# Infini-AI-Lab/Sequoia

Measured on NVIDIA H100. Metric: decoded tokens/sec (mean accepted len/step in config.accepted_tokens_per_step), Sequoia tree speculative decoding, 68m->7B Llama (config c2 unless --config says otherwise), higher is better.
Workload: dtype f16

## Files before the change

sequoia_b200/csrc/sq_gemm.cu:

```cuda
#include <cstdio>
#include <cstdlib>

#include "sq_common.cuh"
#include "sq_ptx.cuh"

struct sq_gemm_plan {
  CUtensorMap tm_a, tm_w;
  __half* c;
  int ldc, n_max, N, K, bn, split, stages, mc, pdl, tiled, epi, n_out;
  int* err_flag;
};

namespace sq {

struct GemmArgs {
  __half* c;
  int ldc, n, N, K, kb_per_split;
  int tiled, kb_total;
  int m0;
  int epi, n_out;
  int* err_flag;
};

constexpr int G_BK = 64;
constexpr int G_THREADS = 384;
constexpr int G_CONSUMER_WARPS = 8;

template <int BN, int STAGES, int SPLIT>
struct GemmSmem {
  static constexpr int A_BYTES = 128 * 128;
  static constexpr int W_BYTES = BN * 128;
  static constexpr int STAGE_BYTES = A_BYTES + ((W_BYTES + 1023) / 1024) * 1024;
  static constexpr int OFF_BAR = STAGES * STAGE_BYTES;
  static constexpr int OFF_RED = OFF_BAR + 256;
  static constexpr int R_STRIDE = BN + 4;
  static constexpr int RED_BYTES = SPLIT > 1 ? 128 * R_STRIDE * 4 : 0;
  static constexpr int TOTAL = OFF_RED + RED_BYTES;
};

__device__ __forceinline__ void tma_load_2d_mc(uint32_t dst, const CUtensorMap* tm, uint32_t bar, int c0, int c1, uint16_t mask) {
  asm volatile(
      "cp.async.bulk.tensor.2d.shared::cluster.global.mbarrier::complete_tx::bytes.multicast::cluster [%0], [%1, {%4, %5}], [%2], %3;" ::"r"(dst),
      "l"(tm), "r"(bar), "h"(mask), "r"(c0), "r"(c1)
      : "memory");
}

template <int BN, int STAGES, int SPLIT, int MC>
__global__ void __launch_bounds__(G_THREADS, 1)
    gemm_tn_kernel(const __grid_constant__ CUtensorMap tm_a, const __grid_constant__ CUtensorMap tm_w, GemmArgs g) {
  using SM = GemmSmem<BN, STAGES, SPLIT>;
  constexpr int NCH = BN / 64;
  extern __shared__ __align__(1024) uint8_t smem_raw[];
  uint8_t* smem = smem_raw + ((1024u - (ptx::smem_u32(smem_raw) & 1023u)) & 1023u);
  const int tid = threadIdx.x, warp = tid >> 5, lane = tid & 31;
  const int n0 = blockIdx.x * BN;
  const int ks = blockIdx.y;
  const int mcr = (MC > 1) ? (int)(blockIdx.x % MC) : 0;
  const int kb0 = ks * g.kb_per_split;
  const int nkb = g.kb_per_split;
  const uint32_t s_base = ptx::smem_u32(smem);
  const uint32_t bar_full = s_base + SM::OFF_BAR, bar_empty = bar_full + 8 * STAGES;

  if (tid == 0) {
#pragma unroll
    for (int s = 0; s < STAGES; ++s) {
      ptx::mbar_init(bar_full + 8 * s, 1);
      ptx::mbar_init(bar_empty + 8 * s, G_CONSUMER_WARPS * MC);
    }
    ptx::fence_barrier_init();
  }
  __syncthreads();
  if (MC > 1)
    asm volatile("barrier.cluster.arrive.release.aligned;\n\tbarrier.cluster.wait.acquire.aligned;" ::: "memory");

  if (warp < 4) {
    if (tid == 0) {
      asm volatile("griddepcontrol.launch_dependents;" ::: "memory");
      const int pre = nkb < STAGES ? nkb : STAGES;
      for (int kb = 0; kb < pre; ++kb) {
        const uint32_t sa = s_base + kb * SM::STAGE_BYTES, sw = sa + SM::A_BYTES;
        ptx::mbar_expect_tx(bar_full + 8 * kb, SM::A_BYTES + SM::W_BYTES);
        if (g.tiled) ptx::tma_load_2d(sw, &tm_w, bar_full + 8 * kb, 0, ((int)blockIdx.x * g.kb_total + kb0 + kb) * BN);
        else ptx::tma_load_2d(sw, &tm_w, bar_full + 8 * kb, (kb0 + kb) * G_BK, n0);
      }
      asm volatile("griddepcontrol.wait;" ::: "memory");
      int stage = 0;
      uint32_t phase = 0;
      for (int kb = 0; kb < nkb; ++kb) {
        const uint32_t sa = s_base + stage * SM::STAGE_BYTES, sw = sa + SM::A_BYTES;
        if (kb >= pre) {
          ptx::mbar_wait_one(bar_empty + 8 * stage, phase ^ 1, g.err_flag, 11);
          ptx::mbar_expect_tx(bar_full + 8 * stage, SM::A_BYTES + SM::W_BYTES);
          if (g.tiled) ptx::tma_load_2d(sw, &tm_w, bar_full + 8 * stage, 0, ((int)blockIdx.x * g.kb_total + kb0 + kb) * BN);
          else ptx::tma_load_2d(sw, &tm_w, bar_full + 8 * stage, (kb0 + kb) * G_BK, n0);
        }
        if (MC == 1) ptx::tma_load_2d(sa, &tm_a, bar_full + 8 * stage, (kb0 + kb) * G_BK, g.m0);
        else tma_load_2d_mc(sa + mcr * (SM::A_BYTES / MC), &tm_a, bar_full + 8 * stage, (kb0 + kb) * G_BK, g.m0 + mcr * (128 / MC),
                            (uint16_t)(((1u << MC) - 1u) << (MC * ks)));
        if (++stage == STAGES) { stage = 0; phase ^= 1; }
      }
    }
  } else {
    const int wg = (warp >> 2) - 1;
    float acc[NCH][32];
#pragma unroll
    for (int c = 0; c < NCH; ++c)
#pragma unroll
      for (int e = 0; e < 32; ++e) acc[c][e] = 0.f;
    auto release = [&](int s) {
      if (lane == 0) {
        if (MC == 1) asm volatile("mbarrier.arrive.shared::cta.b64 _, [%0];" ::"r"(bar_empty + 8 * s) : "memory");
        else
          for (int r = 0; r < MC; ++r) ptx::mbar_arrive_cluster(bar_empty + 8 * s, (uint32_t)(MC * ks + r));
      }
    };
    int stage = 0, prev = -1;
    uint32_t phase = 0;
    for (int kb = 0; kb < nkb; ++kb) {
      ptx::mbar_wait(bar_full + 8 * stage, phase, g.err_flag, 12);
      const uint32_t sa = s_base + stage * SM::STAGE_BYTES + wg * 8192, sw = s_base + stage * SM::STAGE_BYTES + SM::A_BYTES;
      ptx::wgmma_fence();
#pragma unroll
      for (int k = 0; k < G_BK / 16; ++k)
#pragma unroll
        for (int c = 0; c < NCH; ++c)
          ptx::wgmma_ss<0>(acc[c], gmma_desc(sa + k * 32, 16, 1024), gmma_desc(sw + c * 8192 + k * 32, 16, 1024), 1);
      ptx::wgmma_commit();
      asm volatile("wgmma.wait_group.sync.aligned 1;" ::: "memory");
      if (prev >= 0) release(prev);
      prev = stage;
      if (++stage == STAGES) { stage = 0; phase ^= 1; }
    }
    ptx::wgmma_wait_all();
    if (prev >= 0) release(prev);
    const int rbase = wg * 64 + (warp & 3) * 16 + (lane >> 2), q2 = 2 * (lane & 3);
    if (SPLIT == 1 && g.epi == 1) {
#pragma unroll
      for (int h = 0; h < 2; ++h) {
        const int row = rbase + 8 * h;
        if (row >= g.n) continue;
        __half* orow = g.c + (int64_t)(g.m0 + row) * g.ldc;
#pragma unroll
        for (int c = 0; c < NCH; ++c)
#pragma unroll
          for (int j = 0; j < 8; ++j) {
            if ((j & 3) >= 2) continue;
            const int ob = (n0 + c * 64 + (j >> 2) * 32) / 2;
            if (ob >= g.n_out) continue;
            __half o[2];
#pragma unroll
            for (int e = 0; e < 2; ++e) {
              const float x = h2f(f2h(acc[c][4 * j + 2 * h + e]));
              const __half act = f2h(x / (1.0f + expf(-x)));
              o[e] = f2h(h2f(act) * h2f(f2h(acc[c][4 * (j + 2) + 2 * h + e])));
            }
            *reinterpret_cast<__half2*>(orow + ob + (j & 3) * 8 + q2) = __halves2half2(o[0], o[1]);
          }
      }
    } else if (SPLIT == 1) {
#pragma unroll
      for (int h = 0; h < 2; ++h) {
        const int row = rbase + 8 * h;
        if (row >= g.n) continue;
        __half* crow = g.c + (int64_t)(g.m0 + row) * g.ldc + n0;
#pragma unroll
        for (int c = 0; c < NCH; ++c)
#pragma unroll
          for (int j = 0; j < 8; ++j)
            if (n0 + c * 64 + j * 8 < g.N)
              *reinterpret_cast<__half2*>(crow + c * 64 + j * 8 + q2) =
                  __floats2half2_rn(acc[c][4 * j + 2 * h], acc[c][4 * j + 2 * h + 1]);
      }
    } else {
      constexpr int RPC = 128 / SPLIT;
#pragma unroll
      for (int h = 0; h < 2; ++h) {
        const int row = rbase + 8 * h;
        uint32_t dst;
        asm volatile("mapa.shared::cluster.u32 %0, %1, %2;" : "=r"(dst) : "r"(s_base + SM::OFF_RED), "r"((uint32_t)mcr + MC * (row / RPC)));
        dst += (uint32_t)((ks * RPC + row % RPC) * SM::R_STRIDE * 4);
#pragma unroll
        for (int c = 0; c < NCH; ++c)
#pragma unroll
          for (int j = 0; j < 8; ++j)
            asm volatile("st.shared::cluster.v2.f32 [%0], {%1, %2};" ::"r"(dst + (c * 64 + j * 8 + q2) * 4),
                         "f"(acc[c][4 * j + 2 * h]), "f"(acc[c][4 * j + 2 * h + 1])
                         : "memory");
      }
    }
  }
  __syncthreads();

  if (MC > 1 || SPLIT > 1)
    asm volatile("barrier.cluster.arrive.release.aligned;\n\tbarrier.cluster.wait.acquire.aligned;" ::: "memory");

  if (SPLIT > 1) {
    constexpr int RPC = 128 / SPLIT;
    constexpr int CPR = BN / 4;
    const float* red = reinterpret_cast<const float*>(smem + SM::OFF_RED);
    for (int i = tid; i < RPC * CPR; i += G_THREADS) {
      const int lr = i / CPR, cc = i % CPR;
      const int row = ks * RPC + lr;
      if (row >= g.n) continue;
      float4 acc = make_float4(0.f, 0.f, 0.f, 0.f);
#pragma unroll
      for (int s = 0; s < SPLIT; ++s) {
        const float4 o = *reinterpret_cast<const float4*>(red + (s * RPC + lr) * SM::R_STRIDE + cc * 4);
        acc.x += o.x; acc.y += o.y; acc.z += o.z; acc.w += o.w;
      }
      const __half2 lo = __floats2half2_rn(acc.x, acc.y), hi = __floats2half2_rn(acc.z, acc.w);
      uint2 pk;
      pk.x = *reinterpret_cast<const uint32_t*>(&lo);
      pk.y = *reinterpret_cast<const uint32_t*>(&hi);
      *reinterpret_cast<uint2*>(g.c + (int64_t)(g.m0 + row) * g.ldc + n0 + cc * 4) = pk;
    }
  }
}

}

using namespace sq;

typedef CUresult (*PFN_tmapEncodeTiledG)(CUtensorMap*, CUtensorMapDataType, cuuint32_t, void*, const cuuint64_t*,
                                         const cuuint64_t*, const cuuint32_t*, const cuuint32_t*, CUtensorMapInterleave,
                                         CUtensorMapSwizzle, CUtensorMapL2promotion, CUtensorMapFloatOOBfill);

static int encode_2d(CUtensorMap* tm, const void* base, uint64_t inner, uint64_t outer, uint64_t pitch_bytes,
                     uint32_t box_inner, uint32_t box_outer, CUtensorMapL2promotion prom) {
  static PFN_tmapEncodeTiledG fn = nullptr;
  if (!fn) {
    void* p = nullptr;
    cudaDriverEntryPointQueryResult qres;
    if (cudaGetDriverEntryPoint("cuTensorMapEncodeTiled", &p, cudaEnableDefault, &qres) == cudaSuccess &&
        qres == cudaDriverEntryPointSuccess)
      fn = (PFN_tmapEncodeTiledG)p;
  }
  if (!fn) { set_error("cuTensorMapEncodeTiled unavailable"); return SQ_ERR_CUDA; }
  cuuint64_t dims[2] = {inner, outer};
  cuuint64_t strides[1] = {pitch_bytes};
  cuuint32_t box[2] = {box_inner, box_outer};
  cuuint32_t estr[2] = {1, 1};
  CUresult r = fn(tm, CU_TENSOR_MAP_DATA_TYPE_FLOAT16, 2, const_cast<void*>(base), dims, strides, box, estr,
                  CU_TENSOR_MAP_INTERLEAVE_NONE, CU_TENSOR_MAP_SWIZZLE_128B, prom, CU_TENSOR_MAP_FLOAT_OOB_FILL_NONE);
  if (r != CUDA_SUCCESS) { set_error("cuTensorMapEncodeTiled failed: %d", (int)r); return SQ_ERR_CUDA; }
  return SQ_OK;
}

static int sm_count() {
  static int n_sm = 0;
  if (!n_sm) {
    int dev = 0;
    if (cudaGetDevice(&dev) != cudaSuccess || cudaDeviceGetAttribute(&n_sm, cudaDevAttrMultiProcessorCount, dev) != cudaSuccess ||
        n_sm <= 0) {
      cudaGetLastError();
      n_sm = 132;
    }
  }
  return n_sm;
}

static void choose_tiles(sq_gemm_plan* p, bool allow_split) {
  const int N = p->N, kb = p->K / 64;
  const int n_sm = sm_count();
  const int cands[] = {256, 192, 128, 64};
  int best_bn = 128, best_split = 1, best_mc = 1;
  double best_score = -1.0;
  for (int bn : cands) {
    const int tiles = (N + bn - 1) / bn;
    for (int split : {1, 2, 4}) {
      if (kb % split || (split > 1 && !allow_split)) continue;
      if (split > 1 && (bn > 128 || N % bn)) continue;
      const int ctas = tiles * split;
      if (ctas > n_sm) continue;
      for (int mc : {1, 2}) {
        if (mc == 2 && tiles % 2) continue;
        const double a_share = 128.0 / mc, share = bn / (bn + a_share);
        double score = ctas * share;
        if (split > 1) score *= 0.85;
        if (score > best_score) { best_score = score; best_bn = bn; best_split = split; best_mc = mc; }
      }
    }
  }
  p->bn = best_bn; p->split = best_split; p->mc = best_mc;
}

static void pick_tiles(sq_gemm_plan* p) {
  const int kb = p->K / 64;
  const bool allow_split = p->epi == 0;
  choose_tiles(p, allow_split);
  const char* force = getenv("SQ_GEMM_FORCE");
  if (force) {
    int fb = 0, fs = 0, fm = 1;
    const int nf = sscanf(force, "%d,%d,%d", &fb, &fs, &fm);
    const bool bn_ok = fb == 64 || fb == 128 || fb == 192 || fb == 256;
    if (nf >= 2 && bn_ok && (fs == 1 || fs == 2 || fs == 4) && kb % fs == 0 && (fm == 1 || fm == 2) &&
        !(fs > 1 && (fb > 128 || p->N % fb || !allow_split)) && !(fm == 2 && ((p->N + fb - 1) / fb) % 2)) {
      p->bn = fb; p->split = fs; p->mc = fm;
    }
  }
}

extern "C" int sq_gemm_pick_tiles(int N, int K, int* bn, int* split, int* mc) { return sq_gemm_pick_tiles_ex(N, K, 0, bn, split, mc); }

extern "C" int sq_gemm_pick_tiles_ex(int N, int K, int flags, int* bn, int* split, int* mc) {
  SQ_CHECK_ARG(K % 64 == 0 && N % 32 == 0, "sq_gemm_pick_tiles: K %% 64, N %% 32");
  sq_gemm_plan p{};
  p.N = N; p.K = K; p.epi = (flags & SQ_GEMM_SWIGLU) ? 1 : 0;
  pick_tiles(&p);
  *bn = p.bn; *split = p.split; *mc = p.mc;
  return SQ_OK;
}

static int plan_create(sq_gemm_plan** plan, const sq_half* a, int lda, int n_max, const sq_half* w, int N, int K, sq_half* c,
                       int ldc, int* err_flag, int flags);

extern "C" int sq_gemm_plan_create(sq_gemm_plan** plan, const sq_half* a, int lda, int n_max, const sq_half* w, int N,
                                   int K, sq_half* c, int ldc, int* err_flag) {
  return plan_create(plan, a, lda, n_max, w, N, K, c, ldc, err_flag, 0);
}

extern "C" int sq_gemm_plan_create_tiled(sq_gemm_plan** plan, const sq_half* a, int lda, int n_max, const sq_half* w_tiled,
                                         int N, int K, sq_half* c, int ldc, int* err_flag) {
  return plan_create(plan, a, lda, n_max, w_tiled, N, K, c, ldc, err_flag, SQ_GEMM_TILED);
}

extern "C" int sq_gemm_plan_create_ex(sq_gemm_plan** plan, const sq_half* a, int lda, int n_max, const sq_half* w, int N,
                                      int K, sq_half* c, int ldc, int* err_flag, int flags) {
  return plan_create(plan, a, lda, n_max, w, N, K, c, ldc, err_flag, flags);
}

static int plan_create(sq_gemm_plan** plan, const sq_half* a, int lda, int n_max, const sq_half* w, int N, int K, sq_half* c,
                       int ldc, int* err_flag, int flags) {
  const int tiled = (flags & SQ_GEMM_TILED) ? 1 : 0;
  SQ_CHECK_ARG(plan && a && w && c, "sq_gemm_plan_create: null pointer");
  SQ_CHECK_ARG(K % 64 == 0 && N % 32 == 0 && lda % 8 == 0 && ldc % 8 == 0, "sq_gemm_plan_create: K %% 64, N %% 32");
  sq_gemm_plan* p = new sq_gemm_plan();
  p->c = (__half*)c; p->ldc = ldc; p->n_max = n_max; p->N = N; p->K = K; p->err_flag = err_flag;
  p->tiled = tiled; p->epi = (flags & SQ_GEMM_SWIGLU) ? 1 : 0; p->n_out = p->epi ? N / 2 : 0;
  if (p->epi) SQ_CHECK_ARG(N % 32 == 0, "sq_gemm_plan_create: SwiGLU needs N %% 32 == 0");
  pick_tiles(p);
  {
    p->pdl = pdl_enabled() ? 1 : 0;
  }
  p->stages = p->split > 1 ? 4 : (p->bn == 256 ? 4 : p->bn == 192 ? 5 : p->bn == 128 ? 6 : 8);
  int rc = encode_2d(&p->tm_a, a, (uint64_t)K, (uint64_t)n_max, (uint64_t)lda * 2, 64, (uint32_t)(128 / p->mc),
                     CU_TENSOR_MAP_L2_PROMOTION_L2_128B);
  if (!rc) {
    if (tiled) rc = encode_2d(&p->tm_w, w, 64, (uint64_t)((N + p->bn - 1) / p->bn) * (uint64_t)(K / 64) * (uint64_t)p->bn, 128, 64,
                              (uint32_t)p->bn, CU_TENSOR_MAP_L2_PROMOTION_L2_256B);
    else rc = encode_2d(&p->tm_w, w, (uint64_t)K, (uint64_t)N, (uint64_t)K * 2, 64, (uint32_t)p->bn, CU_TENSOR_MAP_L2_PROMOTION_L2_256B);
  }
  if (rc) { delete p; return rc; }
  *plan = p;
  return SQ_OK;
}

extern "C" int sq_gemm_plan_destroy(sq_gemm_plan* plan) {
  delete plan;
  return SQ_OK;
}

template <int BN, int STAGES, int SPLIT, int MC>
static int launch_gemm(sq_gemm_plan* p, GemmArgs& g, cudaStream_t st) {
  using SM = GemmSmem<BN, STAGES, SPLIT>;
  constexpr int smem = SM::TOTAL + 1024;
  static_assert(smem <= 227 * 1024, "shared memory budget");
  static bool attr = false;
  if (!attr) {
    cudaError_t e = cudaFuncSetAttribute(gemm_tn_kernel<BN, STAGES, SPLIT, MC>, cudaFuncAttributeMaxDynamicSharedMemorySize, smem);
    if (e != cudaSuccess) { set_error("sq_gemm: smem attr: %s", cudaGetErrorString(e)); return SQ_ERR_CUDA; }
    attr = true;
  }
  cudaLaunchConfig_t cfg{};
  cfg.gridDim = dim3((p->N + BN - 1) / BN, SPLIT, 1);
  cfg.blockDim = dim3(G_THREADS);
  cfg.dynamicSmemBytes = smem;
  cfg.stream = st;
  cudaLaunchAttribute at[2];
  at[0].id = cudaLaunchAttributeClusterDimension;
  at[0].val.clusterDim.x = MC;
  at[0].val.clusterDim.y = SPLIT;
  at[0].val.clusterDim.z = 1;
  cfg.attrs = at;
  cfg.numAttrs = 1;
  if (p->pdl) {
    at[1].id = cudaLaunchAttributeProgrammaticStreamSerialization;
    at[1].val.programmaticStreamSerializationAllowed = 1;
    cfg.numAttrs = 2;
  }
  cudaError_t e = cudaLaunchKernelEx(&cfg, gemm_tn_kernel<BN, STAGES, SPLIT, MC>, p->tm_a, p->tm_w, g);
  if (e != cudaSuccess) { set_error("sq_gemm: launch failed: %s", cudaGetErrorString(e)); return SQ_ERR_CUDA; }
  SQ_CHECK_LAUNCH("sq_gemm");
  return SQ_OK;
}

static int run_tile(sq_gemm_plan* plan, GemmArgs& g, cudaStream_t st) {
  const int bn = plan->bn, sp = plan->split, mc = plan->mc;
#define SQ_G(BN_, ST_, SP_, MC_) if (bn == BN_ && sp == SP_ && mc == MC_) return launch_gemm<BN_, ST_, SP_, MC_>(plan, g, st)
  SQ_G(256, 4, 1, 1); SQ_G(256, 4, 1, 2);
  SQ_G(192, 5, 1, 1); SQ_G(192, 5, 1, 2);
  SQ_G(128, 6, 1, 1); SQ_G(128, 6, 1, 2); SQ_G(128, 4, 2, 1); SQ_G(128, 4, 4, 1); SQ_G(128, 4, 2, 2); SQ_G(128, 4, 4, 2);
  SQ_G(64, 8, 1, 1); SQ_G(64, 8, 1, 2); SQ_G(64, 4, 2, 1); SQ_G(64, 4, 4, 1); SQ_G(64, 4, 2, 2); SQ_G(64, 4, 4, 2);
#undef SQ_G
  set_error("sq_gemm_run: no kernel for bn=%d split=%d mc=%d", bn, sp, mc);
  return SQ_ERR_UNSUPPORTED;
}

extern "C" int sq_gemm_run(sq_gemm_plan* plan, int n, void* stream) { return sq_gemm_run_at(plan, n, 0, nullptr, 0, stream); }

extern "C" int sq_gemm_run_at(sq_gemm_plan* plan, int n, int a_row0, sq_half* c, int ldc, void* stream) {
  SQ_CHECK_ARG(plan != nullptr, "sq_gemm_run: null plan");
  SQ_CHECK_ARG(n >= 0 && a_row0 >= 0 && a_row0 + n <= plan->n_max, "sq_gemm_run: rows [%d, %d) exceed the plan's n_max=%d", a_row0, a_row0 + n, plan->n_max);
  SQ_CHECK_ARG(c == nullptr || (ldc % 8 == 0 && ((uintptr_t)c % 16) == 0), "sq_gemm_run: output override must be 16 B aligned, pitch %% 8");
  for (int m0 = 0; m0 < n; m0 += 128) {
    GemmArgs g;
    g.n = n - m0 < 128 ? n - m0 : 128; g.N = plan->N; g.K = plan->K;
    g.kb_per_split = plan->K / 64 / plan->split;
    g.tiled = plan->tiled; g.kb_total = plan->K / 64;
    g.m0 = a_row0 + m0; g.epi = plan->epi; g.n_out = plan->n_out;
    if (c) { g.ldc = ldc; g.c = (__half*)c - (int64_t)a_row0 * ldc; }
    else { g.ldc = plan->ldc; g.c = plan->c; }
    g.err_flag = plan->err_flag;
    const int rc = run_tile(plan, g, (cudaStream_t)stream);
    if (rc != SQ_OK) return rc;
  }
  return SQ_OK;
}

extern "C" int sq_gemm_plan_set_epilogue(sq_gemm_plan* plan, int kind, int n_out) {
  SQ_CHECK_ARG(plan != nullptr && (kind == 0 || kind == 1), "sq_gemm_plan_set_epilogue: bad arguments");
  SQ_CHECK_ARG(kind == 0 || (plan->split == 1 && n_out % 16 == 0 && 2 * n_out <= plan->N + 31), "sq_gemm_plan_set_epilogue: SwiGLU needs split 1, n_out %% 16 == 0");
  plan->epi = kind; plan->n_out = n_out;
  return SQ_OK;
}

extern "C" int sq_gemm_plan_info(sq_gemm_plan* plan, int* bn, int* split, int* stages) {
  *bn = plan->bn; *split = plan->split; *stages = plan->stages + 100 * plan->mc;
  return SQ_OK;
}
```

sequoia_b200/csrc/sq_ptx.cuh:

```cuda
#pragma once
#include <cuda.h>

#include "sq_common.cuh"

namespace sq {

namespace ptx {
__device__ __forceinline__ uint32_t smem_u32(const void* p) { return (uint32_t)__cvta_generic_to_shared(p); }
__device__ __forceinline__ void mbar_init(uint32_t bar, uint32_t count) {
  asm volatile("mbarrier.init.shared::cta.b64 [%0], %1;" ::"r"(bar), "r"(count) : "memory");
}
__device__ __forceinline__ void fence_barrier_init() { asm volatile("fence.mbarrier_init.release.cluster;" ::: "memory"); }
__device__ __forceinline__ void mbar_expect_tx(uint32_t bar, uint32_t bytes) {
  asm volatile("mbarrier.arrive.expect_tx.shared::cta.b64 _, [%0], %1;" ::"r"(bar), "r"(bytes) : "memory");
}
__device__ __forceinline__ bool mbar_try_wait(uint32_t bar, uint32_t parity) {
  uint32_t ok;
  asm volatile(
      "{\n\t.reg .pred p;\n\t"
      "mbarrier.try_wait.parity.shared::cta.b64 p, [%1], %2;\n\t"
      "selp.u32 %0, 1, 0, p;\n\t}"
      : "=r"(ok)
      : "r"(bar), "r"(parity)
      : "memory");
  return ok != 0;
}
__device__ __forceinline__ bool mbar_wait(uint32_t bar, uint32_t parity, int* err_flag, int code) {
  const long long t0 = clock64();
  bool ok = false;
  while (!(ok = mbar_try_wait(bar, parity))) {
    if (clock64() - t0 > 2000000000LL) break;
  }
  if (!ok && err_flag) atomicExch(err_flag, code);
  __syncwarp();
  return ok;
}
__device__ __forceinline__ bool mbar_wait_one(uint32_t bar, uint32_t parity, int* err_flag, int code) {
  const long long t0 = clock64();
  bool ok = false;
  while (!(ok = mbar_try_wait(bar, parity))) {
    if (clock64() - t0 > 2000000000LL) break;
  }
  if (!ok && err_flag) atomicExch(err_flag, code);
  return ok;
}
__device__ __forceinline__ void tma_load_2d(uint32_t dst, const CUtensorMap* tm, uint32_t bar, int c0, int c1) {
  asm volatile(
      "cp.async.bulk.tensor.2d.shared::cluster.global.mbarrier::complete_tx::bytes [%0], [%1, {%3, %4}], [%2];" ::"r"(dst),
      "l"(tm), "r"(bar), "r"(c0), "r"(c1)
      : "memory");
}
__device__ __forceinline__ void tma_load_3d(uint32_t dst, const CUtensorMap* tm, uint32_t bar, int c0, int c1, int c2) {
  asm volatile(
      "cp.async.bulk.tensor.3d.shared::cluster.global.mbarrier::complete_tx::bytes [%0], [%1, {%3, %4, %5}], [%2];" ::"r"(
          dst),
      "l"(tm), "r"(bar), "r"(c0), "r"(c1), "r"(c2)
      : "memory");
}
__device__ __forceinline__ void mbar_arrive_cluster(uint32_t bar, uint32_t cta) {
  asm volatile(
      "{\n\t.reg .b32 ra;\n\tmapa.shared::cluster.u32 ra, %0, %1;\n\t"
      "mbarrier.arrive.release.cluster.shared::cluster.b64 _, [ra];\n\t}" ::"r"(bar), "r"(cta)
      : "memory");
}
__device__ __forceinline__ void wgmma_fence() { asm volatile("wgmma.fence.sync.aligned;" ::: "memory"); }
__device__ __forceinline__ void wgmma_commit() { asm volatile("wgmma.commit_group.sync.aligned;" ::: "memory"); }
__device__ __forceinline__ void wgmma_wait_all() { asm volatile("wgmma.wait_group.sync.aligned 0;" ::: "memory"); }
template <int TB>
__device__ __forceinline__ void wgmma_ss(float (&d)[32], uint64_t adesc, uint64_t bdesc, uint32_t accum) {
  asm volatile(
      "{\n\t.reg .pred p;\n\tsetp.ne.b32 p, %34, 0;\n\t"
      "wgmma.mma_async.sync.aligned.m64n64k16.f32.f16.f16 {%0,%1,%2,%3,%4,%5,%6,%7,%8,%9,%10,%11,%12,%13,%14,%15,%16,%17,%18,%19,%20,%21,%22,%23,%24,%25,%26,%27,%28,%29,%30,%31}, %32, %33, p, 1, 1, 0, %35;\n\t}"
      : "+f"(d[0]), "+f"(d[1]), "+f"(d[2]), "+f"(d[3]), "+f"(d[4]), "+f"(d[5]), "+f"(d[6]), "+f"(d[7]), "+f"(d[8]), "+f"(d[9]), "+f"(d[10]), "+f"(d[11]), "+f"(d[12]), "+f"(d[13]), "+f"(d[14]), "+f"(d[15]), "+f"(d[16]), "+f"(d[17]), "+f"(d[18]), "+f"(d[19]), "+f"(d[20]), "+f"(d[21]), "+f"(d[22]), "+f"(d[23]), "+f"(d[24]), "+f"(d[25]), "+f"(d[26]), "+f"(d[27]), "+f"(d[28]), "+f"(d[29]), "+f"(d[30]), "+f"(d[31])
      : "l"(adesc), "l"(bdesc), "r"(accum), "n"(TB)
      : "memory");
}
template <int TB>
__device__ __forceinline__ void wgmma_rs(float (&d)[32], const uint32_t (&a)[4], uint64_t bdesc, uint32_t accum) {
  asm volatile(
      "{\n\t.reg .pred p;\n\tsetp.ne.b32 p, %37, 0;\n\t"
      "wgmma.mma_async.sync.aligned.m64n64k16.f32.f16.f16 {%0,%1,%2,%3,%4,%5,%6,%7,%8,%9,%10,%11,%12,%13,%14,%15,%16,%17,%18,%19,%20,%21,%22,%23,%24,%25,%26,%27,%28,%29,%30,%31}, {%32, %33, %34, %35}, %36, p, 1, 1, %38;\n\t}"
      : "+f"(d[0]), "+f"(d[1]), "+f"(d[2]), "+f"(d[3]), "+f"(d[4]), "+f"(d[5]), "+f"(d[6]), "+f"(d[7]), "+f"(d[8]), "+f"(d[9]), "+f"(d[10]), "+f"(d[11]), "+f"(d[12]), "+f"(d[13]), "+f"(d[14]), "+f"(d[15]), "+f"(d[16]), "+f"(d[17]), "+f"(d[18]), "+f"(d[19]), "+f"(d[20]), "+f"(d[21]), "+f"(d[22]), "+f"(d[23]), "+f"(d[24]), "+f"(d[25]), "+f"(d[26]), "+f"(d[27]), "+f"(d[28]), "+f"(d[29]), "+f"(d[30]), "+f"(d[31])
      : "r"(a[0]), "r"(a[1]), "r"(a[2]), "r"(a[3]), "l"(bdesc), "r"(accum), "n"(TB)
      : "memory");
}
}

__device__ __forceinline__ uint64_t gmma_desc(uint32_t smem_addr, uint32_t lbo_bytes, uint32_t sbo_bytes) {
  uint64_t d = 0;
  d |= (uint64_t)((smem_addr & 0x3FFFFu) >> 4);
  d |= (uint64_t)((lbo_bytes >> 4) & 0x3FFFu) << 16;
  d |= (uint64_t)((sbo_bytes >> 4) & 0x3FFFu) << 32;
  d |= (uint64_t)1 << 62;
  return d;
}

}
```

sequoia_b200/model.py:

```python
from __future__ import annotations

import json
import math
import os
from dataclasses import dataclass
from typing import Dict, Optional

import torch

from . import ops

F16 = torch.float16


@dataclass
class LlamaConfigLite:
    hidden_size: int
    intermediate_size: int
    num_hidden_layers: int
    num_attention_heads: int
    num_key_value_heads: int
    vocab_size: int = 32000
    rms_norm_eps: float = 1e-6
    rope_theta: float = 10000.0
    max_position_embeddings: int = 2048
    rope_scaling: Optional[dict] = None

    @property
    def head_dim(self):
        return self.hidden_size // self.num_attention_heads


NAMED_CONFIGS = {
    "llama-68m": LlamaConfigLite(768, 3072, 2, 12, 12),
    "llama-160m": LlamaConfigLite(768, 3072, 12, 12, 12),
    "llama-2-7b": LlamaConfigLite(4096, 11008, 32, 32, 32, rms_norm_eps=1e-5, max_position_embeddings=4096),
    "llama-2-13b": LlamaConfigLite(5120, 13824, 40, 40, 40, rms_norm_eps=1e-5, max_position_embeddings=4096),
    "llama-2-70b": LlamaConfigLite(8192, 28672, 80, 64, 8, rms_norm_eps=1e-5, max_position_embeddings=4096),
    "llama-2-70b-8l": LlamaConfigLite(8192, 28672, 8, 64, 8, rms_norm_eps=1e-5, max_position_embeddings=4096),
    "llama-3.2-1b": LlamaConfigLite(2048, 8192, 16, 32, 8, vocab_size=128256, rms_norm_eps=1e-5, rope_theta=500000.0,
                                    max_position_embeddings=131072,
                                    rope_scaling=dict(rope_type="llama3", factor=32.0, low_freq_factor=1.0,
                                                      high_freq_factor=4.0, original_max_position_embeddings=8192)),
    "llama-3.1-8b": LlamaConfigLite(4096, 14336, 32, 32, 8, vocab_size=128256, rms_norm_eps=1e-5, rope_theta=500000.0,
                                    max_position_embeddings=131072,
                                    rope_scaling=dict(rope_type="llama3", factor=8.0, low_freq_factor=1.0,
                                                      high_freq_factor=4.0, original_max_position_embeddings=8192)),
}


def parse_rope_scaling(rs) -> Optional[dict]:
    if rs is None:
        return None
    kind = rs.get("rope_type", rs.get("type"))
    if kind in (None, "default"):
        return None
    if kind != "llama3":
        raise ValueError(f"rope_scaling type {kind!r} is not supported (supported: None, 'llama3')")
    return dict(rope_type="llama3", factor=float(rs["factor"]), low_freq_factor=float(rs["low_freq_factor"]),
                high_freq_factor=float(rs["high_freq_factor"]),
                original_max_position_embeddings=int(rs["original_max_position_embeddings"]))


def llama3_inv_freq(inv_freq: torch.Tensor, rs: dict) -> torch.Tensor:
    factor, lo, hi = rs["factor"], rs["low_freq_factor"], rs["high_freq_factor"]
# ... 159 lines not shown
    def __init__(self, model_name_or_path, max_length: int, device="cuda:0", tp_group=None, n_max: Optional[int] = None,
                 batch_size: int = 1, weight_format: str = "fp16"):
        if weight_format not in ("fp16", "fp8"):
            raise ValueError(f"weight_format must be 'fp16' or 'fp8', got {weight_format!r}")
        if weight_format == "fp8" and tp_group is not None:
            raise NotImplementedError("FP8 target weights run on one GPU: tensor parallelism needs weight_format='fp16'")
        self.weight_format = weight_format
        self.device = torch.device(device)
        self.B = batch_size
        self.cfg, src = resolve_model(model_name_or_path, self.device)
        cfg = self.cfg
        self.tp = TPInfo(tp_group)
        tp, r = self.tp.size, self.tp.rank
        assert cfg.num_attention_heads % tp == 0 and cfg.num_key_value_heads % tp == 0 and cfg.intermediate_size % tp == 0
        self.M = max_length
        self.n_max = n_max or max_length * batch_size
        self.H, self.Hkv, self.D = cfg.num_attention_heads // tp, cfg.num_key_value_heads // tp, cfg.head_dim
        self.I = cfg.intermediate_size // tp
        h, D, V = cfg.hidden_size, self.D, cfg.vocab_size
        self.h, self.V, self.L = h, V, cfg.num_hidden_layers
        if weight_format == "fp8":
            shapes = (((self.H + 2 * self.Hkv) * D, h), (h, self.H * D), (2 * self.I, h), (h, self.I))
            if any(n % 64 or k % 64 for n, k in shapes):
                raise ValueError(f"weight_format='fp8' needs every layer projection (N, K) to be multiples of 64, got {shapes}")
        wts = load_sharded_weights(cfg, src, r, tp)
        self.embed, self.layers, self.norm, self.lm_head = wts["embed"], wts["layers"], wts["norm"], wts["lm_head"]
        self.cos, self.sin = rope_cache(cfg, max_length, self.device)
        self.eps = float(cfg.rms_norm_eps)
        n = self.n_max
        dev = self.device
        z = lambda *s: torch.zeros(*s, dtype=F16, device=dev)
        self.hidden, self.normed = z(n, h), z(n, h)
        self.qkv = z(n, (self.H + 2 * self.Hkv) * D)
        self.attn_out, self.proj = z(n, self.H * D), z(n, h)
        self.gate_up, self.act = z(n, 2 * self.I), z(n, self.I)
        self.logits = z(n, V)
        self.k_cache = torch.zeros(self.L, batch_size, self.Hkv, max_length, D, dtype=F16, device=dev)
        self.v_cache = torch.zeros_like(self.k_cache)
        self.plan = ops.AttnPlan(self.qkv, n, self.H, self.Hkv, D, self.k_cache, self.v_cache, self.attn_out)
        self.gemm_err = torch.zeros(4, dtype=torch.int32, device=dev)
        self.lm_plan = None
        if weight_format == "fp8":
            io = dict(wqkv=(self.normed, self.qkv), wo=(self.attn_out, self.proj), wgu=(self.normed, self.gate_up),
                      wd=(self.act, self.proj))
            for ly in self.layers:
                for k in self.PROJECTIONS:
                    q, s = ops.quantize_fp8(ly.pop(k))
                    ly[k + "_fp8"] = ops.GemmFp8Plan(io[k][0], q, s, io[k][1], self.gemm_err)
                    del q
            torch.cuda.empty_cache()
        stream_sized = h >= 2048
        ok = stream_sized and tp == 1 and weight_format == "fp16" and self.I % 16 == 0 and h % 64 == 0
        self.gu_interleaved = False
        if ok and ops.gemm_pick_tiles(2 * self.I, h, ops.GEMM_SWIGLU)[2] == 1:
            self.gu_interleaved = True
            for ly in self.layers:
                ly["wgu"] = ops.interleave_gate_up(ly["wgu"][:self.I], ly["wgu"][self.I:])
                ly["wgu_plan"] = ops.GemmPlan(self.normed, ly["wgu"], self.act, self.gemm_err, swiglu=True)
        if stream_sized and V % 32 == 0 and h % 64 == 0:
            self.lm_plan = ops.GemmPlan(self.normed, self.lm_head, self.logits, self.gemm_err)
        self.draft_plan = None
        if (os.environ.get("SQ_DRAFT_ATTN", "1") != "0" and tp == 1 and batch_size == 1 and
                ops.draft_supported(h, self.H, self.Hkv, D, max_length)):
            self.draft_plan = ops.DraftPlan(h, self.L, self.H, max_length, self.k_cache, self.v_cache)
        self.peer = None
        if self.tp.size > 1 and os.environ.get("SQ_TP_MODE", "fused") == "fused":
            from .peer import PeerBuffers
            self.peer = PeerBuffers(tp_group, self.device, n, h)

    def _gate_up_act(self, ly, n: int):
        plan = ly.get("wgu_plan")
        if plan is not None and 96 < n <= 128:
            plan.run(n)
            return
        self._project(ly, "wgu", self.normed, n, self.gate_up)
        ops.silu_mul(self.gate_up, self.act, n, interleaved=self.gu_interleaved)

    def _project(self, ly, k: str, a: torch.Tensor, n: int, out: torch.Tensor):
        plan = ly.get(k + "_fp8")
        if plan is not None:
            plan.run(n)
        else:
            torch.mm(a[:n], ly[k].t(), out=out[:n])

    def weight_bytes(self) -> int:
        b = 2 * (self.embed.numel() + self.lm_head.numel() + self.norm.numel())
        for ly in self.layers:
            b += 2 * (ly["ln1"].numel() + ly["ln2"].numel())
            b += sum(ly[k + "_fp8"].weight_bytes() if k + "_fp8" in ly else 2 * ly[k].numel() for k in self.PROJECTIONS)
        return b

    @torch.no_grad()
    def forward(self, n: int, tokens: torch.Tensor, position_ids: torch.Tensor, storage_ids: torch.Tensor, *,
                state=None, n0: int = 0, kv_end: int = 0, prefix_len: int = 0, dense_mask=None, mask_ld: int = 0,
                tree_bits=None, tree_words: int = 0, tree_size: int = 0, logits_out: Optional[torch.Tensor] = None,
                logits_from: int = 0, skip_lm_head: bool = False, batch: bool = False,
                logits_to: Optional[int] = None) -> Optional[torch.Tensor]:
        B = self.B if batch else 1
        N = n * B
        assert 0 < N <= self.n_max
        assert not batch or (state is not None and dense_mask is None)
        H, Hkv, D, M = self.H, self.Hkv, self.D, self.M
        small = (not batch and self.draft_plan is not None and state is not None and n <= ops.DraftPlan.MAX_ROWS
                 and dense_mask is None)
        if batch:
            ops.embed_rows_batch(self.embed, tokens, n, self.hidden, state, n0=n0)
        else:
            ops.embed_rows(self.embed, tokens, n, self.hidden, state=state, n0=n0)
        n_seq = n

        def attend(l):
            if batch:
                ops.rope_kv_append_batch(self.qkv, H, Hkv, D, self.cos, self.sin, position_ids, storage_ids, n_seq,
                                         self.k_cache[l], self.v_cache[l], M, state, n0=n0)
                ops.tree_attn_batch(self.plan, l, n_seq, state=state, n0=n0, kv_end=kv_end, tree_bits=tree_bits,
                                    tree_words=tree_words, tree_size=tree_size)
                return
            ops.rope_kv_append(self.qkv, H, Hkv, D, self.cos, self.sin, position_ids, storage_ids, n, self.k_cache[l],
                               self.v_cache[l], M, state=state, n0=n0)
            if small:
                self.draft_plan.attention(l, n, self.qkv, self.attn_out, state, n0, kv_end, tree_bits, tree_words,
                                          tree_size)
            else:
                ops.tree_attn(self.plan, l, n, state=state, n0=n0, kv_end=kv_end, prefix_len=prefix_len,
                              dense_mask=dense_mask, mask_ld=mask_ld, tree_bits=tree_bits, tree_words=tree_words,
                              tree_size=tree_size)

        self._layers(N, attend)
        if skip_lm_head:
            return None
        return self._lm_head(logits_from, N if logits_to is None else logits_to, logits_out)

# ... 54 lines not shown
```

Measured before the change: 202.7.

## Drop multicast tiles, size split-K by cluster occupancy, always interleave gate/up

The tile chooser no longer considers 2-CTA multicast for the A operand. It now limits split-K candidates by the resident cluster count from cudaOccupancyMaxActiveClusters and requires at least 32 k-blocks per split. Because multicast is never chosen, gate/up weights are now always interleaved for the fused SwiGLU GEMM on the 7B model. Cluster barrier and remote mbarrier arrives also drop their release semantics, which could weaken memory ordering where split-K clusters exchange partial sums.

New measurement: 201.1 (median of 6 runs). About the same (-0.8%).

```diff
diff --git a/sequoia_b200/csrc/sq_gemm.cu b/sequoia_b200/csrc/sq_gemm.cu
--- a/sequoia_b200/csrc/sq_gemm.cu
+++ b/sequoia_b200/csrc/sq_gemm.cu
@@ -71,7 +71,7 @@
   }
   __syncthreads();
   if (MC > 1)
-    asm volatile("barrier.cluster.arrive.release.aligned;\n\tbarrier.cluster.wait.acquire.aligned;" ::: "memory");
+    asm volatile("barrier.cluster.arrive.relaxed.aligned;\n\tbarrier.cluster.wait.acquire.aligned;" ::: "memory");
 
   if (warp < 4) {
     if (tid == 0) {
@@ -259,29 +259,51 @@
   return n_sm;
 }
 
+static int resident_ctas(int cs) {
+  static int cache[9] = {0};
+  if (cs <= 1) return sm_count();
+  if (!cache[cs]) {
+    auto fn = gemm_tn_kernel<64, 4, 2, 1>;
+    const int smem = GemmSmem<64, 4, 2>::TOTAL + 1024;
+    cudaLaunchConfig_t cfg{};
+    cudaLaunchAttribute at[1];
+    cfg.gridDim = dim3(cs, 1, 1);
+    cfg.blockDim = dim3(G_THREADS);
+    cfg.dynamicSmemBytes = smem;
+    at[0].id = cudaLaunchAttributeClusterDimension;
+    at[0].val.clusterDim.x = cs; at[0].val.clusterDim.y = 1; at[0].val.clusterDim.z = 1;
+    cfg.attrs = at;
+    cfg.numAttrs = 1;
+    int n = 0;
+    if (cudaFuncSetAttribute(fn, cudaFuncAttributeMaxDynamicSharedMemorySize, smem) == cudaSuccess &&
+        cudaOccupancyMaxActiveClusters(&n, fn, &cfg) == cudaSuccess && n > 0) {
+      cache[cs] = n * cs;
+    } else {
+      cudaGetLastError();
+      cache[cs] = cs == 2 ? 132 : 120;
+    }
+  }
+  return cache[cs];
+}
+
 static void choose_tiles(sq_gemm_plan* p, bool allow_split) {
   const int N = p->N, kb = p->K / 64;
-  const int n_sm = sm_count();
   const int cands[] = {256, 192, 128, 64};
-  int best_bn = 128, best_split = 1, best_mc = 1;
+  int best_bn = 128, best_split = 1;
   double best_score = -1.0;
   for (int bn : cands) {
     const int tiles = (N + bn - 1) / bn;
     for (int split : {1, 2, 4}) {
       if (kb % split || (split > 1 && !allow_split)) continue;
-      if (split > 1 && (bn > 128 || N % bn)) continue;
+      if (split > 1 && (bn > 128 || N % bn || kb / split < 32)) continue;
       const int ctas = tiles * split;
-      if (ctas > n_sm) continue;
-      for (int mc : {1, 2}) {
-        if (mc == 2 && tiles % 2) continue;
-        const double a_share = 128.0 / mc, share = bn / (bn + a_share);
-        double score = ctas * share;
-        if (split > 1) score *= 0.85;
-        if (score > best_score) { best_score = score; best_bn = bn; best_split = split; best_mc = mc; }
-      }
-    }
-  }
-  p->bn = best_bn; p->split = best_split; p->mc = best_mc;
+      if (ctas > resident_ctas(split)) continue;
+      double score = ctas * (bn / (bn + 128.0));
+      if (split > 1) score *= 0.85;
+      if (score > best_score) { best_score = score; best_bn = bn; best_split = split; }
+    }
+  }
+  p->bn = best_bn; p->split = best_split; p->mc = 1;
 }
 
 static void pick_tiles(sq_gemm_plan* p) {
diff --git a/sequoia_b200/csrc/sq_ptx.cuh b/sequoia_b200/csrc/sq_ptx.cuh
--- a/sequoia_b200/csrc/sq_ptx.cuh
+++ b/sequoia_b200/csrc/sq_ptx.cuh
@@ -60,7 +60,7 @@
 __device__ __forceinline__ void mbar_arrive_cluster(uint32_t bar, uint32_t cta) {
   asm volatile(
       "{\n\t.reg .b32 ra;\n\tmapa.shared::cluster.u32 ra, %0, %1;\n\t"
-      "mbarrier.arrive.release.cluster.shared::cluster.b64 _, [ra];\n\t}" ::"r"(bar), "r"(cta)
+      "mbarrier.arrive.shared::cluster.b64 _, [ra];\n\t}" ::"r"(bar), "r"(cta)
       : "memory");
 }
 __device__ __forceinline__ void wgmma_fence() { asm volatile("wgmma.fence.sync.aligned;" ::: "memory"); }
diff --git a/sequoia_b200/model.py b/sequoia_b200/model.py
--- a/sequoia_b200/model.py
+++ b/sequoia_b200/model.py
@@ -276,7 +276,7 @@
         stream_sized = h >= 2048
         ok = stream_sized and tp == 1 and weight_format == "fp16" and self.I % 16 == 0 and h % 64 == 0
         self.gu_interleaved = False
-        if ok and ops.gemm_pick_tiles(2 * self.I, h, ops.GEMM_SWIGLU)[2] == 1:
+        if ok:
             self.gu_interleaved = True
             for ly in self.layers:
                 ly["wgu"] = ops.interleave_gate_up(ly["wgu"][:self.I], ly["wgu"][self.I:])
```

## Route down projection through split-K custom GEMM with ring-reused reduction smem

Applied to the files above, without the earlier changes.

Adds a 'deep' split-K GEMM variant that reuses the pipeline ring buffers for the split-K reduction, so it can keep full stage depth. It also adds L2 cache hints (evict-first for weights, evict-last for activations), drops split-4 and multicast-with-split from tile selection, and relaxes the cluster arrive ordering. The model now uses the custom GEMM for the wd projection at verify sizes (96<n<=128) when the tile picker selects bn=64/split=2, instead of torch.mm. Optional timestamp probes are compiled in only under a macro. Risks include extra cluster barriers and a changed memory-ordering semantic on the cluster arrive.

Result: faster. 203.2 before, 210.5 after (median of 6 runs) (+3.6%).

```diff
diff --git a/sequoia_b200/csrc/sq_gemm.cu b/sequoia_b200/csrc/sq_gemm.cu
--- a/sequoia_b200/csrc/sq_gemm.cu
+++ b/sequoia_b200/csrc/sq_gemm.cu
@@ -8,7 +8,12 @@
   CUtensorMap tm_a, tm_w;
   __half* c;
   int ldc, n_max, N, K, bn, split, stages, mc, pdl, tiled, epi, n_out;
+  int deep;
   int* err_flag;
+#ifdef SQ_GEMM_STAMPS
+  unsigned long long* stamps;
+  int max_clusters;
+#endif
 };
 
 namespace sq {
@@ -20,23 +25,60 @@
   int m0;
   int epi, n_out;
   int* err_flag;
+#ifdef SQ_GEMM_STAMPS
+  unsigned long long* stamps;
+#endif
 };
+
+#ifdef SQ_GEMM_STAMPS
+__device__ __forceinline__ unsigned long long globaltimer() {
+  unsigned long long t;
+  asm volatile("mov.u64 %0, %globaltimer;" : "=l"(t));
+  return t;
+}
+#define SQ_STAMP(slot, value) \
+  do { if (g.stamps) g.stamps[(blockIdx.y * gridDim.x + blockIdx.x) * 5 + (slot)] = (value); } while (0)
+#else
+#define SQ_STAMP(slot, value) do { } while (0)
+#endif
 
 constexpr int G_BK = 64;
 constexpr int G_THREADS = 384;
 constexpr int G_CONSUMER_WARPS = 8;
 
-template <int BN, int STAGES, int SPLIT>
+template <int BN, int STAGES, int SPLIT, bool RING_RED = false>
 struct GemmSmem {
   static constexpr int A_BYTES = 128 * 128;
   static constexpr int W_BYTES = BN * 128;
   static constexpr int STAGE_BYTES = A_BYTES + ((W_BYTES + 1023) / 1024) * 1024;
   static constexpr int OFF_BAR = STAGES * STAGE_BYTES;
-  static constexpr int OFF_RED = OFF_BAR + 256;
+  static constexpr int OFF_RED = RING_RED ? 0 : OFF_BAR + 256;
   static constexpr int R_STRIDE = BN + 4;
   static constexpr int RED_BYTES = SPLIT > 1 ? 128 * R_STRIDE * 4 : 0;
-  static constexpr int TOTAL = OFF_RED + RED_BYTES;
+  static constexpr int TOTAL = RING_RED ? OFF_BAR + 256 : OFF_RED + RED_BYTES;
+  static_assert(!RING_RED || RED_BYTES <= OFF_BAR, "reduction slots must fit in the ring");
 };
+
+__device__ __forceinline__ void cluster_arrive_wait() {
+  asm volatile("barrier.cluster.arrive.release;\n\tbarrier.cluster.wait.acquire;" ::: "memory");
+}
+
+__device__ __forceinline__ uint64_t l2_policy_evict_first() {
+  uint64_t p;
+  asm volatile("createpolicy.fractional.L2::evict_first.b64 %0, 1.0;" : "=l"(p));
+  return p;
+}
+__device__ __forceinline__ uint64_t l2_policy_evict_last() {
+  uint64_t p;
+  asm volatile("createpolicy.fractional.L2::evict_last.b64 %0, 1.0;" : "=l"(p));
+  return p;
+}
+__device__ __forceinline__ void tma_load_2d_hint(uint32_t dst, const CUtensorMap* tm, uint32_t bar, int c0, int c1, uint64_t policy) {
+  asm volatile(
+      "cp.async.bulk.tensor.2d.shared::cluster.global.mbarrier::complete_tx::bytes.L2::cache_hint [%0], [%1, {%3, %4}], [%2], %5;" ::"r"(dst),
+      "l"(tm), "r"(bar), "r"(c0), "r"(c1), "l"(policy)
+      : "memory");
+}
 
 __device__ __forceinline__ void tma_load_2d_mc(uint32_t dst, const CUtensorMap* tm, uint32_t bar, int c0, int c1, uint16_t mask) {
   asm volatile(
@@ -45,10 +87,10 @@
       : "memory");
 }
 
-template <int BN, int STAGES, int SPLIT, int MC>
-__global__ void __launch_bounds__(G_THREADS, 1)
-    gemm_tn_kernel(const __grid_constant__ CUtensorMap tm_a, const __grid_constant__ CUtensorMap tm_w, GemmArgs g) {
-  using SM = GemmSmem<BN, STAGES, SPLIT>;
+template <int BN, int STAGES, int SPLIT, int MC, bool RING_RED>
+__device__ __forceinline__ void gemm_tn_body(const CUtensorMap& tm_a, const CUtensorMap& tm_w, GemmArgs g) {
+  static_assert(!RING_RED || (SPLIT > 1 && MC == 1), "ring reduction: split-K without multicast");
+  using SM = GemmSmem<BN, STAGES, SPLIT, RING_RED>;
   constexpr int NCH = BN / 64;
   extern __shared__ __align__(1024) uint8_t smem_raw[];
   uint8_t* smem = smem_raw + ((1024u - (ptx::smem_u32(smem_raw) & 1023u)) & 1023u);
@@ -76,12 +118,19 @@
   if (warp < 4) {
     if (tid == 0) {
       asm volatile("griddepcontrol.launch_dependents;" ::: "memory");
+#ifdef SQ_GEMM_STAMPS
+      uint32_t smid;
+      asm volatile("mov.u32 %0, %smid;" : "=r"(smid));
+      SQ_STAMP(0, smid);
+      SQ_STAMP(1, globaltimer());
+#endif
+      const uint64_t pol_w = l2_policy_evict_first(), pol_a = l2_policy_evict_last();
       const int pre = nkb < STAGES ? nkb : STAGES;
       for (int kb = 0; kb < pre; ++kb) {
         const uint32_t sa = s_base + kb * SM::STAGE_BYTES, sw = sa + SM::A_BYTES;
         ptx::mbar_expect_tx(bar_full + 8 * kb, SM::A_BYTES + SM::W_BYTES);
-        if (g.tiled) ptx::tma_load_2d(sw, &tm_w, bar_full + 8 * kb, 0, ((int)blockIdx.x * g.kb_total + kb0 + kb) * BN);
-        else ptx::tma_load_2d(sw, &tm_w, bar_full + 8 * kb, (kb0 + kb) * G_BK, n0);
+        if (g.tiled) tma_load_2d_hint(sw, &tm_w, bar_full + 8 * kb, 0, ((int)blockIdx.x * g.kb_total + kb0 + kb) * BN, pol_w);
+        else tma_load_2d_hint(sw, &tm_w, bar_full + 8 * kb, (kb0 + kb) * G_BK, n0, pol_w);
       }
       asm volatile("griddepcontrol.wait;" ::: "memory");
       int stage = 0;
@@ -91,15 +140,16 @@
         if (kb >= pre) {
           ptx::mbar_wait_one(bar_empty + 8 * stage, phase ^ 1, g.err_flag, 11);
           ptx::mbar_expect_tx(bar_full + 8 * stage, SM::A_BYTES + SM::W_BYTES);
-          if (g.tiled) ptx::tma_load_2d(sw, &tm_w, bar_full + 8 * stage, 0, ((int)blockIdx.x * g.kb_total + kb0 + kb) * BN);
-          else ptx::tma_load_2d(sw, &tm_w, bar_full + 8 * stage, (kb0 + kb) * G_BK, n0);
+          if (g.tiled) tma_load_2d_hint(sw, &tm_w, bar_full + 8 * stage, 0, ((int)blockIdx.x * g.kb_total + kb0 + kb) * BN, pol_w);
+          else tma_load_2d_hint(sw, &tm_w, bar_full + 8 * stage, (kb0 + kb) * G_BK, n0, pol_w);
         }
-        if (MC == 1) ptx::tma_load_2d(sa, &tm_a, bar_full + 8 * stage, (kb0 + kb) * G_BK, g.m0);
+        if (MC == 1) tma_load_2d_hint(sa, &tm_a, bar_full + 8 * stage, (kb0 + kb) * G_BK, g.m0, pol_a);
         else tma_load_2d_mc(sa + mcr * (SM::A_BYTES / MC), &tm_a, bar_full + 8 * stage, (kb0 + kb) * G_BK, g.m0 + mcr * (128 / MC),
                             (uint16_t)(((1u << MC) - 1u) << (MC * ks)));
         if (++stage == STAGES) { stage = 0; phase ^= 1; }
       }
     }
+    if constexpr (RING_RED) cluster_arrive_wait();
   } else {
     const int wg = (warp >> 2) - 1;
     float acc[NCH][32];
@@ -118,6 +168,10 @@
     uint32_t phase = 0;
     for (int kb = 0; kb < nkb; ++kb) {
       ptx::mbar_wait(bar_full + 8 * stage, phase, g.err_flag, 12);
+#ifdef SQ_GEMM_STAMPS
+      if (tid == 128 && kb == 0) SQ_STAMP(2, globaltimer());
+      if (tid == 128 && kb == nkb - 1) SQ_STAMP(3, globaltimer());
+#endif
       const uint32_t sa = s_base + stage * SM::STAGE_BYTES + wg * 8192, sw = s_base + stage * SM::STAGE_BYTES + SM::A_BYTES;
       ptx::wgmma_fence();
 #pragma unroll
@@ -133,6 +187,7 @@
     }
     ptx::wgmma_wait_all();
     if (prev >= 0) release(prev);
+    if constexpr (RING_RED) cluster_arrive_wait();
     const int rbase = wg * 64 + (warp & 3) * 16 + (lane >> 2), q2 = 2 * (lane & 3);
     if (SPLIT == 1 && g.epi == 1) {
 #pragma unroll
@@ -215,6 +270,22 @@
       *reinterpret_cast<uint2*>(g.c + (int64_t)(g.m0 + row) * g.ldc + n0 + cc * 4) = pk;
     }
   }
+#ifdef SQ_GEMM_STAMPS
+  __syncthreads();
+  if (tid == 0) SQ_STAMP(4, globaltimer());
+#endif
+}
+
+template <int BN, int STAGES, int SPLIT, int MC>
+__global__ void __launch_bounds__(G_THREADS, 1)
+    gemm_tn_kernel(const __grid_constant__ CUtensorMap tm_a, const __grid_constant__ CUtensorMap tm_w, GemmArgs g) {
+  gemm_tn_body<BN, STAGES, SPLIT, MC, false>(tm_a, tm_w, g);
+}
+
+template <int BN, int STAGES, int SPLIT>
+__global__ void __launch_bounds__(G_THREADS, 1)
+    gemm_tn_deep_kernel(const __grid_constant__ CUtensorMap tm_a, const __grid_constant__ CUtensorMap tm_w, GemmArgs g) {
+  gemm_tn_body<BN, STAGES, SPLIT, 1, true>(tm_a, tm_w, g);
 }
 
 }
@@ -267,13 +338,13 @@
   double best_score = -1.0;
   for (int bn : cands) {
     const int tiles = (N + bn - 1) / bn;
-    for (int split : {1, 2, 4}) {
+    for (int split : {1, 2}) {
       if (kb % split || (split > 1 && !allow_split)) continue;
       if (split > 1 && (bn > 128 || N % bn)) continue;
       const int ctas = tiles * split;
       if (ctas > n_sm) continue;
       for (int mc : {1, 2}) {
-        if (mc == 2 && tiles % 2) continue;
+        if (mc == 2 && (tiles % 2 || split > 1)) continue;
         const double a_share = 128.0 / mc, share = bn / (bn + a_share);
         double score = ctas * share;
         if (split > 1) score *= 0.85;
@@ -282,6 +353,7 @@
     }
   }
   p->bn = best_bn; p->split = best_split; p->mc = best_mc;
+  p->deep = best_split > 1;
 }
 
 static void pick_tiles(sq_gemm_plan* p) {
@@ -290,12 +362,13 @@
   choose_tiles(p, allow_split);
   const char* force = getenv("SQ_GEMM_FORCE");
   if (force) {
-    int fb = 0, fs = 0, fm = 1;
-    const int nf = sscanf(force, "%d,%d,%d", &fb, &fs, &fm);
+    int fb = 0, fs = 0, fm = 1, fd = 0;
+    const int nf = sscanf(force, "%d,%d,%d,%d", &fb, &fs, &fm, &fd);
     const bool bn_ok = fb == 64 || fb == 128 || fb == 192 || fb == 256;
     if (nf >= 2 && bn_ok && (fs == 1 || fs == 2 || fs == 4) && kb % fs == 0 && (fm == 1 || fm == 2) &&
         !(fs > 1 && (fb > 128 || p->N % fb || !allow_split)) && !(fm == 2 && ((p->N + fb - 1) / fb) % 2)) {
       p->bn = fb; p->split = fs; p->mc = fm;
+      p->deep = nf == 4 && fd == 1 && fs == 2 && fm == 1;
     }
   }
 }
@@ -342,7 +415,7 @@
   {
     p->pdl = pdl_enabled() ? 1 : 0;
   }
-  p->stages = p->split > 1 ? 4 : (p->bn == 256 ? 4 : p->bn == 192 ? 5 : p->bn == 128 ? 6 : 8);
+  p->stages = p->split > 1 && !p->deep ? 4 : (p->bn == 256 ? 4 : p->bn == 192 ? 5 : p->bn == 128 ? 6 : 8);
   int rc = encode_2d(&p->tm_a, a, (uint64_t)K, (uint64_t)n_max, (uint64_t)lda * 2, 64, (uint32_t)(128 / p->mc),
                      CU_TENSOR_MAP_L2_PROMOTION_L2_128B);
   if (!rc) {
@@ -360,14 +433,18 @@
   return SQ_OK;
 }
 
-template <int BN, int STAGES, int SPLIT, int MC>
+template <int BN, int STAGES, int SPLIT, int MC, bool DEEP = false>
 static int launch_gemm(sq_gemm_plan* p, GemmArgs& g, cudaStream_t st) {
-  using SM = GemmSmem<BN, STAGES, SPLIT>;
+  using SM = GemmSmem<BN, STAGES, SPLIT, DEEP>;
   constexpr int smem = SM::TOTAL + 1024;
   static_assert(smem <= 227 * 1024, "shared memory budget");
+  static_assert(!DEEP || MC == 1, "gemm_tn_deep_kernel has no multicast");
+  void (*kernel)(CUtensorMap, CUtensorMap, GemmArgs);
+  if constexpr (DEEP) kernel = gemm_tn_deep_kernel<BN, STAGES, SPLIT>;
+  else kernel = gemm_tn_kernel<BN, STAGES, SPLIT, MC>;
   static bool attr = false;
   if (!attr) {
-    cudaError_t e = cudaFuncSetAttribute(gemm_tn_kernel<BN, STAGES, SPLIT, MC>, cudaFuncAttributeMaxDynamicSharedMemorySize, smem);
+    cudaError_t e = cudaFuncSetAttribute(kernel, cudaFuncAttributeMaxDynamicSharedMemorySize, smem);
     if (e != cudaSuccess) { set_error("sq_gemm: smem attr: %s", cudaGetErrorString(e)); return SQ_ERR_CUDA; }
     attr = true;
   }
@@ -388,7 +465,17 @@
     at[1].val.programmaticStreamSerializationAllowed = 1;
     cfg.numAttrs = 2;
   }
-  cudaError_t e = cudaLaunchKernelEx(&cfg, gemm_tn_kernel<BN, STAGES, SPLIT, MC>, p->tm_a, p->tm_w, g);
+#ifdef SQ_GEMM_STAMPS
+  if (p->max_clusters < 0) {
+    cfg.numAttrs = 1;
+    if (cudaOccupancyMaxActiveClusters(&p->max_clusters, kernel, &cfg) != cudaSuccess) {
+      cudaGetLastError();
+      p->max_clusters = -2;
+    }
+    return SQ_OK;
+  }
+#endif
+  cudaError_t e = cudaLaunchKernelEx(&cfg, kernel, p->tm_a, p->tm_w, g);
   if (e != cudaSuccess) { set_error("sq_gemm: launch failed: %s", cudaGetErrorString(e)); return SQ_ERR_CUDA; }
   SQ_CHECK_LAUNCH("sq_gemm");
   return SQ_OK;
@@ -403,6 +490,13 @@
   SQ_G(64, 8, 1, 1); SQ_G(64, 8, 1, 2); SQ_G(64, 4, 2, 1); SQ_G(64, 4, 4, 1); SQ_G(64, 4, 2, 2); SQ_G(64, 4, 4, 2);
 #undef SQ_G
   set_error("sq_gemm_run: no kernel for bn=%d split=%d mc=%d", bn, sp, mc);
+  return SQ_ERR_UNSUPPORTED;
+}
+
+static int run_deep_tile(sq_gemm_plan* plan, GemmArgs& g, cudaStream_t st) {
+  if (plan->bn == 64 && plan->split == 2) return launch_gemm<64, 8, 2, 1, true>(plan, g, st);
+  if (plan->bn == 128 && plan->split == 2) return launch_gemm<128, 6, 2, 1, true>(plan, g, st);
+  set_error("sq_gemm_run: no deep-ring kernel for bn=%d split=%d", plan->bn, plan->split);
   return SQ_ERR_UNSUPPORTED;
 }
 
@@ -421,7 +515,10 @@
     if (c) { g.ldc = ldc; g.c = (__half*)c - (int64_t)a_row0 * ldc; }
     else { g.ldc = plan->ldc; g.c = plan->c; }
     g.err_flag = plan->err_flag;
-    const int rc = run_tile(plan, g, (cudaStream_t)stream);
+#ifdef SQ_GEMM_STAMPS
+    g.stamps = plan->stamps;
+#endif
+    const int rc = plan->deep ? run_deep_tile(plan, g, (cudaStream_t)stream) : run_tile(plan, g, (cudaStream_t)stream);
     if (rc != SQ_OK) return rc;
   }
   return SQ_OK;
@@ -438,3 +535,18 @@
   *bn = plan->bn; *split = plan->split; *stages = plan->stages + 100 * plan->mc;
   return SQ_OK;
 }
+
+#ifdef SQ_GEMM_STAMPS
+extern "C" int sq_gemm_probe_set_stamps(sq_gemm_plan* plan, unsigned long long* stamps) {
+  plan->stamps = stamps;
+  return SQ_OK;
+}
+extern "C" int sq_gemm_probe_max_clusters(sq_gemm_plan* plan, int* max_clusters) {
+  plan->max_clusters = -1;
+  GemmArgs g{};
+  const int rc = run_tile(plan, g, nullptr);
+  *max_clusters = plan->max_clusters;
+  plan->max_clusters = 0;
+  return rc;
+}
+#endif
diff --git a/sequoia_b200/csrc/sq_ptx.cuh b/sequoia_b200/csrc/sq_ptx.cuh
--- a/sequoia_b200/csrc/sq_ptx.cuh
+++ b/sequoia_b200/csrc/sq_ptx.cuh
@@ -60,7 +60,7 @@
 __device__ __forceinline__ void mbar_arrive_cluster(uint32_t bar, uint32_t cta) {
   asm volatile(
       "{\n\t.reg .b32 ra;\n\tmapa.shared::cluster.u32 ra, %0, %1;\n\t"
-      "mbarrier.arrive.release.cluster.shared::cluster.b64 _, [ra];\n\t}" ::"r"(bar), "r"(cta)
+      "mbarrier.arrive.shared::cluster.b64 _, [ra];\n\t}" ::"r"(bar), "r"(cta)
       : "memory");
 }
 __device__ __forceinline__ void wgmma_fence() { asm volatile("wgmma.fence.sync.aligned;" ::: "memory"); }
diff --git a/sequoia_b200/model.py b/sequoia_b200/model.py
--- a/sequoia_b200/model.py
+++ b/sequoia_b200/model.py
@@ -11,6 +11,7 @@
 from . import ops
 
 F16 = torch.float16
+VERIFY_PLANS = {"wd": (64, 2)}
 
 
 @dataclass
@@ -281,6 +282,13 @@
             for ly in self.layers:
                 ly["wgu"] = ops.interleave_gate_up(ly["wgu"][:self.I], ly["wgu"][self.I:])
                 ly["wgu_plan"] = ops.GemmPlan(self.normed, ly["wgu"], self.act, self.gemm_err, swiglu=True)
+        if ok:
+            io = dict(wqkv=(self.normed, self.qkv), wo=(self.attn_out, self.proj), wd=(self.act, self.proj))
+            for k, tile in VERIFY_PLANS.items():
+                if ops.gemm_pick_tiles(*self.layers[0][k].shape)[:2] != tile:
+                    continue
+                for ly in self.layers:
+                    ly[k + "_plan"] = ops.GemmPlan(io[k][0], ly[k], io[k][1], self.gemm_err)
         if stream_sized and V % 32 == 0 and h % 64 == 0:
             self.lm_plan = ops.GemmPlan(self.normed, self.lm_head, self.logits, self.gemm_err)
         self.draft_plan = None
@@ -302,6 +310,8 @@
 
     def _project(self, ly, k: str, a: torch.Tensor, n: int, out: torch.Tensor):
         plan = ly.get(k + "_fp8")
+        if plan is None and 96 < n <= 128:
+            plan = ly.get(k + "_plan")
         if plan is not None:
             plan.run(n)
         else:
```
